# brocksam/pycollo

Measured on AMD Instinct MI355X. Metric: NLP-callback evals/sec (g + jac_g + hess), higher is better.
Workload: dtype f64; 1 GPU; hypersensitive, 1 phase, 2000 mesh sections x 6 Lobatto nodes = 10001 collocation nodes; num_x=20003, num_c=10001, nnz_jac=140003, nnz_hess=20002, tiles=167, threads_per_block=64, waves_per_tile=4, launches_per_eval=1, lds_bytes_per_workgroup=24144, launch_thread_cpu=245, pin_survived_hip_init=True

## Files before the change

pycollo_amd/codegen.py:

```python
from __future__ import annotations

import hashlib
import os
import shutil
import subprocess

import sympy as sym
from sympy.printing.c import C99CodePrinter

from .model import Model, PhaseModel, PointModel

CSRC = os.path.join(os.path.dirname(os.path.abspath(__file__)), "csrc")
CACHE = os.path.join(os.path.dirname(os.path.abspath(__file__)), "_cache")
ARCH = "gfx950"


class _Printer(C99CodePrinter):

    def _print_Pow(self, expr):
        base, exp = expr.base, expr.exp
        b = self.parenthesize(base, 200)
        if exp.is_Integer:
            n = int(exp)
            if n == 0:
# ... 468 lines not shown
        return 2 + len(_static_w_list(model.phases[0], single_phase=True))
    return 3 + len(sorted(set.intersection(*[set(_static_w_list(pm)) for pm in model.phases])))


def part_paths(code_object: str) -> list[str]:
    out, k = [code_object], 1
    while os.path.exists(f"{code_object[:-6]}.p{k}.hsaco"):
        out.append(f"{code_object[:-6]}.p{k}.hsaco")
        k += 1
    return out


def _waves_per_eu() -> int:
    try:
        return int(os.environ.get("PYCOLLO_AMD_WAVES_PER_EU", "0"))
    except ValueError:
        return 0


def _extra_defines() -> list[str]:
    return [d for d in os.environ.get("PYCOLLO_AMD_DEFINES", "").split() if d]


HEAVY_SCRATCH_LIMIT = int(os.environ.get("PYCOLLO_AMD_HEAVY_SCRATCH_LIMIT", "384"))


def _heavy_cap_enabled() -> bool:
    return os.environ.get("PYCOLLO_AMD_HEAVY_CAP", "1") != "0" and _waves_per_eu() == 0


def _heavy_attr(heavy: bool, cap: bool) -> str:
    return "__attribute__((amdgpu_waves_per_eu(2))) " if (heavy and cap) else ""


def _occupancy_attr() -> str:
    w = _waves_per_eu()
    return f"__attribute__((amdgpu_waves_per_eu({w},{w}))) " if w > 0 else ""


def _fp_contract() -> str:
    v = os.environ.get("PYCOLLO_AMD_FP_CONTRACT", "off").strip().lower()
    return v if v in ("off", "fast", "on") else "off"


def _preload_count() -> int:
    try:
        return max(0, int(os.environ.get("PYCOLLO_AMD_PRELOAD", "10")))
    except ValueError:
        return 10


def _kernels_stamp() -> str:
    h = hashlib.sha256()
    for fn in ("pc_kernels.hpp", "pc_solution.hpp", "pc_args.h"):
        with open(os.path.join(CSRC, fn), "rb") as f:
            h.update(f.read())
    with open(os.path.abspath(__file__), "rb") as f:
        h.update(f.read())
    h.update(b"flags:-O3 -ffp-contract=off")
    return h.hexdigest()[:12]


def hipcc_path() -> str | None:
    for cand in (shutil.which("hipcc"), "/opt/rocm/bin/hipcc"):
        if cand and os.path.exists(cand):
            return cand
    return None


def _orders_tag(model: Model, orders, mixed=None) -> str:
    orders = tuple(int(o) for o in orders) if orders is not None else tuple(0 for _ in model.phases)
    if len(orders) != len(model.phases):
        raise ValueError("one section order (or 0) per phase is required")
    tag = "n" + "_".join(str(o) for o in orders)
    mixed = _norm_mixed(model, orders, mixed)
    if any(mixed):
        tag += "-m" + "_".join(".".join(str(n) for n in m) if m else "x" for m in mixed)
    return tag


def code_object_path(model: Model, orders=None, mixed=None) -> str:
    occ = f"_w{_waves_per_eu()}" if _waves_per_eu() > 0 else ""
    if _fp_contract() != "off":
        occ += "_fc" + _fp_contract()
    if _preload_count() != 10:
        occ += f"_pl{_preload_count()}"
    if not _heavy_cap_enabled() and _waves_per_eu() == 0:
        occ += "_nocap"
    if not _heavy_w4_enabled():
        occ += "_nohw4"
    if HEAVY_SCRATCH_LIMIT != 384:
        occ += f"_sl{HEAVY_SCRATCH_LIMIT}"
    if _extra_defines():
        occ += "_d" + hashlib.sha256(" ".join(_extra_defines()).encode()).hexdigest()[:8]
    return os.path.join(CACHE, f"model_{model.digest}_{_kernels_stamp()}_{_orders_tag(model, orders, mixed)}{occ}.hsaco")


def build_code_object(model: Model, orders=None, force: bool = False, verbose: bool = False, mixed=None) -> str:
    os.makedirs(CACHE, exist_ok=True)
    out = code_object_path(model, orders, mixed)
    if os.path.exists(out) and not force:
        return out
    hipcc = hipcc_path()
    if hipcc is None:
        raise RuntimeError(f"code object {out} is not built and hipcc is not available to build it")
    preload = os.environ.get("LD_PRELOAD", "")
    if "rocprof" in preload or any(k.startswith(("ROCPROF", "ROCPROFILER")) for k in os.environ):
# ... 100 lines not shown
```

pycollo_amd/csrc/pc_kernels.hpp:

```cpp
#pragma once

#include <hip/hip_runtime.h>
#include <tuple>
#include <type_traits>
#include <utility>

#include "pc_args.h"

namespace pc {

template <int I>
using ic = std::integral_constant<int, I>;

template <int B, int E, class F>
__device__ __forceinline__ void static_for(F&& f) {
  if constexpr (B < E) {
    f(ic<B>{});
    static_for<B + 1, E>(f);
  }
}

#ifndef PC_SPLIT_MIN
#define PC_SPLIT_MIN 90
#endif

template <class M>
struct S {
  static constexpr int NY = M::NY, NU = M::NU, NZ = M::NY + M::NU, NQ = M::NQ, NP = M::NP, NS = M::NS;
  static constexpr int NT = (M::T0_FREE ? 1 : 0) + (M::TF_FREE ? 1 : 0);
  static constexpr int NFN = NY + NP + NQ, NV = NZ + NS, NJ = M::NJ, NH = M::NH;

  static constexpr int jidx(int r, int c) {
    for (int e = 0; e < NJ; ++e)
      if (M::jr(e) == r && M::jc(e) == c) return e;
    return -1;
  }
  static constexpr bool dep(int r, int c) { return jidx(r, c) >= 0; }
  static constexpr int D(int a) {
    int n = 0;
    for (int b = 0; b < NZ; ++b) n += dep(a, b) ? 1 : 0;
    return n;
  }
  static constexpr int ndep_before(int a, int b) {
    int n = 0;
    for (int bb = 0; bb < b; ++bb) n += dep(a, bb) ? 1 : 0;
    return n;
  }
  static constexpr bool own_sparse(int a) { return !dep(a, a); }
  static constexpr bool is_t(int l) { return M::wk(l) == 2; }
  static constexpr bool is_q(int l) { return M::wk(l) == 1; }
  static constexpr int NWT = [] {
    int n = 0;
    for (int l = 0; l < NS; ++l) n += is_t(l) ? 1 : 0;
    return n;
  }();
  static constexpr int tpar(int jt) {
    for (int l = 0; l < NS; ++l)
      if (is_t(l) && M::wi(l) == jt) return l;
    return -1;
  }
  static constexpr int qpar(int m) {
    for (int l = 0; l < NS; ++l)
      if (is_q(l) && M::wi(l) == m) return l;
    return -1;
  }
  static constexpr int nsdep(int r) {
    int n = 0;
    for (int l = 0; l < NS; ++l) n += dep(r, NZ + l) ? 1 : 0;
    return n;
  }
  static constexpr int srank(int r, int l) {
    int n = 0;
    for (int ll = 0; ll < l; ++ll) n += dep(r, NZ + ll) ? 1 : 0;
    return n;
  }
  static constexpr int nqdep(int r) {
// ... 57 lines not shown
      if (!(r >= NY && r < NY + NP) && dep(r, c)) return true;
    return false;
  }
  static constexpr int hidx(int r, int c) {
    for (int e = 0; e < NH; ++e)
      if (M::hr(e) == r && M::hc(e) == c) return e;
    return -1;
  }
  static constexpr bool tzx(int c) {
    if (tz(c)) return true;
    for (int l = 0; l < NS; ++l)
      if (is_t(l) && hidx(NZ + l, c) >= 0) return true;
    return false;
  }
  static constexpr int erank(int i) {
    int n = 0;
    for (int k = 0; k < i; ++k) n += M::efl(k) ? 1 : 0;
    return n;
  }
  static constexpr int R_Q = 0;
  static constexpr bool has_rts(int l) { return NT > 0 && tz(NZ + l); }
  static constexpr int rqs(int m, int l) {
    int n = NQ;
    for (int mm = 0; mm < NQ; ++mm)
      for (int ll = 0; ll < NS; ++ll) {
        if (mm == m && ll == l) return n;
        n += dep(NY + NP + mm, NZ + ll) ? 1 : 0;
      }
    return n;
  }
  static constexpr int rts(int l) {
    int n = rqs(NQ, 0);
    for (int ll = 0; ll < l; ++ll) n += has_rts(ll) ? 1 : 0;
    return n;
  }
  static constexpr int rss(int l, int l2) {
    int n = rts(NS);
    for (int e = 0; e < NH; ++e)
      if (M::hc(e) >= NZ) {
        if (M::hr(e) == NZ + l && M::hc(e) == NZ + l2) return n;
        ++n;
      }
    return n;
  }
  static constexpr int NRED = rss(NS, NS);
  static constexpr int O_VZ = 0, O_RZ = NZ, O_VQ = 2 * NZ, O_RQ = 2 * NZ + NQ, O_VT = 2 * NZ + 2 * NQ,
                       O_RT = O_VT + 2, O_VS = O_RT + 2, O_RS = O_VS + NS, O_WD = O_RS + NS, O_WP = O_WD + NY,
                       O_WI = O_WP + NP, NSCAL = O_WI + NQ;
  static constexpr int GO_D = 0, GO_P = NY, GO_Q = NY + NP;
  static constexpr int HO_Z = 0, HO_T = NZ, HO_S = 3 * NZ;

  static constexpr int IT_D = 0, IT_P = NY, IT_Q = NY + NP, IT_HB = NY + NP + NQ, IT_HS = IT_HB + NZ,
                       IT_HT = IT_HS + NZ, IT_HSUM = IT_HT + NZ, NITEMS = IT_HSUM + 1;
  struct Deal {
    int own[NITEMS];
    unsigned hmask;
  };
  template <int W, int NN>
  static constexpr Deal deal() {
    Deal d{};
    int wt[NITEMS] = {};
    bool done[NITEMS] = {};
    for (int a = 0; a < NY; ++a) wt[IT_D + a] = D(a) * NN + C(a) + 1;
    for (int m = 0; m < NP; ++m) wt[IT_P + m] = nzdep(NY + m) + nsdep(NY + m) + 1;
    for (int m = 0; m < NQ; ++m) wt[IT_Q + m] = nzdep(NY + NP + m) + 1;
    for (int b = 0; b < NZ; ++b) {
      wt[IT_HB + b] = hrow_count(b) > 0 ? hrow_count(b) + 1 : 0;
      int ns = 0;
      for (int e = 0; e < NH; ++e) ns += (M::hr(e) >= NZ && !is_t(M::hr(e) - NZ) && M::hc(e) == b) ? 1 : 0;
      wt[IT_HS + b] = ns;
      wt[IT_HT + b] = tzx(b) ? NT : 0;
    }
    wt[IT_HSUM] = NS > 0 ? NS + NS * (NS + 1) / 2 : 0;
    int load[W] = {};
    d.hmask = 0;
    for (int it = 0; it < NITEMS; ++it) {
      int best = -1;
      for (int i = 0; i < NITEMS; ++i)
        if (!done[i] && (best < 0 || wt[i] > wt[best])) best = i;
      done[best] = true;
      const bool hess = best >= IT_HB;
      int bin = hess ? W - 1 : 0;
      for (int k = 0; k < W; ++k) {
        const int b = hess ? W - 1 - k : k;
        if (load[b] < load[bin]) bin = b;
      }
      d.own[best] = wt[best] > 0 ? bin : 0;
      load[bin] += wt[best];
      if (hess && wt[best] > 0) d.hmask |= 1u << bin;
    }
    return d;
  }
  static constexpr int red_item(int r) {
    if (r < NQ) return IT_Q + r;
    for (int m = 0; m < NQ; ++m)
      for (int l = 0; l < NS; ++l)
        if (dep(NY + NP + m, NZ + l) && rqs(m, l) == r) return IT_Q + m;
    return IT_HSUM;
  }
};


template <int CTRL>
__device__ __forceinline__ double dpp_mov(double v) {
  const long long b = __builtin_bit_cast(long long, v);
  const int lo = __builtin_amdgcn_update_dpp(0, (int)(b & 0xffffffffll), CTRL, 0xf, 0xf, true);
  const int hi = __builtin_amdgcn_update_dpp(0, (int)(b >> 32), CTRL, 0xf, 0xf, true);
  return __builtin_bit_cast(double, ((long long)(unsigned)hi << 32) | (long long)(unsigned)lo);
}
__device__ __forceinline__ double wave_sum(double v) {
  v += dpp_mov<0x111>(v);
  v += dpp_mov<0x112>(v);
  v += dpp_mov<0x114>(v);
  v += dpp_mov<0x118>(v);
  const long long b = __builtin_bit_cast(long long, v);
  double tot = 0.0;
#pragma unroll
  for (int r = 0; r < 4; ++r) {
    const int lo = __builtin_amdgcn_readlane((int)(b & 0xffffffffll), 16 * r + 15);
    const int hi = __builtin_amdgcn_readlane((int)(b >> 32), 16 * r + 15);
    tot += __builtin_bit_cast(double, ((long long)(unsigned)hi << 32) | (long long)(unsigned)lo);
  }
  return tot;
}

__device__ __forceinline__ void lds_barrier() {
  asm volatile("s_waitcnt lgkmcnt(0)\n\ts_barrier" ::: "memory");
}

typedef double pc_d2_a8 __attribute__((ext_vector_type(2), aligned(8)));
#ifndef PC_FLUSH_DEPTH
#define PC_FLUSH_DEPTH 4
#endif
typedef int pc_i4 __attribute__((ext_vector_type(4)));
__device__ __forceinline__ void flush_run(double* __restrict__ dst, const double* __restrict__ src, int len, int tid,
                                          int TB) {
  len = __builtin_amdgcn_readfirstlane(len);
  if (len <= 0) return;
  const unsigned long long d64 = (unsigned long long)dst;
  double* base = (double*)(((unsigned long long)(unsigned)__builtin_amdgcn_readfirstlane((int)(d64 >> 32)) << 32) |
                           (unsigned long long)(unsigned)__builtin_amdgcn_readfirstlane((int)d64));
  __amdgpu_buffer_rsrc_t rs = __builtin_amdgcn_make_buffer_rsrc(base, 0, len * 8, 0x00020000);
  const int pairs = (len + 1) >> 1;
  const pc_d2_a8* sp = reinterpret_cast<const pc_d2_a8*>(src) + tid;
// ... 9 lines not shown
  }
  if (b0 < pairs) {
    pc_d2_a8 a[PC_FLUSH_DEPTH];
#pragma unroll
    for (int q = 0; q < PC_FLUSH_DEPTH; ++q) a[q] = sp[b0 + q * TB];
#pragma unroll
    for (int q = 0; q < PC_FLUSH_DEPTH; ++q)
      if (b0 + q * TB < pairs)
        __builtin_amdgcn_raw_buffer_store_b128(__builtin_bit_cast(pc_i4, a[q]), rs, voff + q * TB * 16, 0, 0);
  }
}

template <int L, int GS>
__device__ __forceinline__ void flush_chunks(double* __restrict__ dst, const double* __restrict__ src, int nq, int t, int TN) {
  nq = __builtin_amdgcn_readfirstlane(nq);
  if (nq <= 0) return;
  if (TN == 64) {
    constexpr int NR = (L + 127) / 128;
    const unsigned long long d64 = (unsigned long long)dst;
    double* base = (double*)(((unsigned long long)(unsigned)__builtin_amdgcn_readfirstlane((int)(d64 >> 32)) << 32) |
                             (unsigned long long)(unsigned)__builtin_amdgcn_readfirstlane((int)d64));
    const double* sp = src + 2 * t;
    const int voff = 16 * t;
    pc_d2_a8 a[NR], nx[NR];
    auto fetch = [&](pc_d2_a8* r, const double* p) {
#pragma unroll
      for (int i = 0; i < NR; ++i) r[i] = *reinterpret_cast<const pc_d2_a8*>(p + 128 * i);
    };
    auto store = [&](const pc_d2_a8* r, double* b) {
      __amdgpu_buffer_rsrc_t rs = __builtin_amdgcn_make_buffer_rsrc(b, 0, L * 8, 0x00020000);
#pragma unroll
      for (int i = 0; i < NR; ++i) __builtin_amdgcn_raw_buffer_store_b128(__builtin_bit_cast(pc_i4, r[i]), rs, voff + 1024 * i, 0, 0);
    };
    fetch(a, sp);
    int q = 0;
    for (; q + 2 <= nq; q += 2) {
      fetch(nx, sp + L);
      store(a, base);
      if (q + 2 < nq) fetch(a, sp + 2 * L);
      store(nx, base + GS);
      sp += 2 * L;
      base += 2 * GS;
    }
    if (q < nq) store(a, base);
    return;
  }
  for (int q = 0; q < nq; ++q) {
    const double* sp = src + (long long)q * L;
    double* dp = dst + (long long)q * GS;
    for (int o = 2 * t; o < L; o += 2 * TN) {
      if (o + 1 < L) *reinterpret_cast<pc_d2_a8*>(dp + o) = *reinterpret_cast<const pc_d2_a8*>(sp + o);
      else dp[o] = sp[o];
    }
  }
}

template <class St>
struct BulkIn {
  const double* x; const double* lam; double* c; double* G; double* H;
  const double* xz; const double* lamd;
  const int32_t* tile_k0; const int32_t* tile_n0; const int32_t* sec_s; const double* sec_h; const int64_t* sec_E;
  const double* qa; const double* qw; const int64_t* hslot0; const int64_t* hslotN; double* partials;
  unsigned long long* gran; unsigned long long* erec; const double* tab;
  int64_t x_off, s_off, c_off, c_path_off, c_int_off;
  double t_fixed[2];
  int32_t N, K, flags, qa_total, qw_total, tile_begin, uni_n, spt, lds_out, wpt, n_blocks, block_threads, qa0, qw0, qwabs;
  uint32_t epoch;
  int32_t erec0;
  double scal[St::NSCAL > 0 ? St::NSCAL : 1];
  int64_t goff[St::NFN > 0 ? St::NFN : 1];
  int64_t hoff[3 * St::NZ + St::NS * St::NZ > 0 ? 3 * St::NZ + St::NS * St::NZ : 1];
};

#ifndef PC_PIN_BUDGET
#define PC_PIN_BUDGET 40
#endif
template <class T>
__device__ __forceinline__ uintptr_t pin_word(T* v) { return reinterpret_cast<uintptr_t>(v); }
__device__ __forceinline__ unsigned long long pin_word(double v) { return __builtin_bit_cast(unsigned long long, v); }
__device__ __forceinline__ long long pin_word(long long v) { return v; }
__device__ __forceinline__ long pin_word(long v) { return v; }
__device__ __forceinline__ int pin_word(int v) { return v; }
template <class... T>
__device__ __forceinline__ auto pin_vals(const T&... v) { return std::make_tuple(pin_word(v)...); }
template <bool C, class... T>
__device__ __forceinline__ auto pin_if(const T&... v) {
  if constexpr (C) return pin_vals(v...);
  else return std::tuple<>{};
}
template <class Pred, class T, int N, int... I>
__device__ __forceinline__ auto pin_array_impl(const T (&a)[N], std::integer_sequence<int, I...>) {
  return std::tuple_cat(pin_if<Pred::test(I)>(a[I])...);
}
struct PinEvery { static constexpr bool test(int) { return true; } };
template <int CNT, class Pred, class T, int N>
__device__ __forceinline__ auto pin_array_where(const T (&a)[N]) {
  return pin_array_impl<Pred>(a, std::make_integer_sequence<int, CNT>{});
}
template <int CNT, class T, int N>
__device__ __forceinline__ auto pin_array(const T (&a)[N]) { return pin_array_where<CNT, PinEvery>(a); }
#define PC_PIN_OP(i) "s"(std::get<i>(g))
#define PC_PIN_OPS_1 PC_PIN_OP(0)
#define PC_PIN_OPS_2 PC_PIN_OPS_1, PC_PIN_OP(1)
#define PC_PIN_OPS_3 PC_PIN_OPS_2, PC_PIN_OP(2)
#define PC_PIN_OPS_4 PC_PIN_OPS_3, PC_PIN_OP(3)
#define PC_PIN_OPS_5 PC_PIN_OPS_4, PC_PIN_OP(4)
// ... 261 lines not shown
      if (odd_prev) r_cp = tid < r_nprev - 1 ? A.qa[r_qaprev + tid * r_nprev + r_nprev - 1] : 0.0;
    }
  };
  const bool early_aux = LD != nullptr && UN > 0 && !MIX;
  if (early_aux) aux_loads();
  const auto first_group = std::tuple_cat(
      pin_vals(A.x, A.lam, A.sec_h, A.qa, A.qw, A.x_off, A.c_off, A.N, A.K, A.flags, A.qa_total, A.qw_total, A.tile_begin,
               A.uni_n, A.spt, A.lds_out, A.wpt, A.n_blocks, A.block_threads),
      pin_if<(UN > 0)>(A.qa0, A.qwabs), pin_if<(NP > 0)>(A.c_path_off), pin_if<(NQ > 0)>(A.c_int_off), pin_if<(NS > 0)>(A.s_off),
      pin_if<UN == 0>(A.tile_k0, A.tile_n0, A.sec_s, A.sec_E));
  if (early_aux) pin_group<true>(first_group);
  else pin_group(first_group);
  constexpr int NHO = 3 * NZ + NS * NZ;
  constexpr bool PINNED = 2 * (St::NSCAL + NFN + NHO) <= PC_PIN_BUDGET;
  struct ScalUsed {
    static constexpr bool test(int i) {
      return (i < St::O_VQ) || (i >= St::O_VT && i < St::O_VT + St::NT) || (i >= St::O_RT && i < St::O_RT + St::NT) || (i >= St::O_VS);
    }
  };
  struct HoffUsed {
    static constexpr bool test(int i) { return i < St::NZ || (St::NT > 0 && i < 3 * St::NZ) || i >= 3 * St::NZ; }
  };
  auto pin_second_group = [&]() {
    auto outs = std::tuple_cat(pin_vals(A.c, A.G, A.H), pin_if<(NRED > 0 && RES)>(A.gran), pin_if<(NRED > 0 && !RES)>(A.partials),
                               pin_if<!M::T0_FREE>(A.t_fixed[0]), pin_if<!M::TF_FREE>(A.t_fixed[1]));
    if constexpr (PINNED) {
      pin_group(std::tuple_cat(outs, pin_array_where<St::NSCAL, ScalUsed>(A.scal), pin_array<NFN>(A.goff),
                               pin_array_where<NHO, HoffUsed>(A.hoff)));
    } else {
      pin_group(std::tuple_cat(outs, pin_vals(A.tab)));
    }
  };

  extern __shared__ double smem[];
  const int TN = W > 1 ? 64 : TB;
  const int w = WN > 0 ? WIDX : (W > 1 ? __builtin_amdgcn_readfirstlane(tid >> 6) : 0);
  const LdsPlan lp = lds_plan(TN, A.qa_total, A.qw_total, NY, NFS, NRED, A.lds_out * W, St::NSCAL + NFN + 3 * NZ + NS * NZ, UN == 0, MIX);
  double* s_cp = smem + lp.cp;
  double* s_qa = smem + lp.qa;
  double* s_qw = smem + lp.qw;
  int* s_off = reinterpret_cast<int*>(smem + lp.off);
  auto QAO = [&](int n) -> int { return UN > 0 ? 0 : s_off[n]; };
  auto QWO = [&](int n) -> int { return UN > 0 ? 0 : s_off[PC_MAX_ORDER + 1 + n]; };
  double* s_h = smem + lp.h;
  long long* s_E = reinterpret_cast<long long*>(smem + lp.E);
  int* s_s = reinterpret_cast<int*>(smem + lp.s);
  int* s_kr = reinterpret_cast<int*>(smem + lp.kr);
  double* s_f = smem + lp.f;
  double* s_yu = smem + lp.yu;
  double* s_fs = smem + lp.fs;
  double* s_lam = smem + lp.lam;
  double* s_red = smem + lp.red;
  double* s_out = smem + lp.out + w * A.lds_out;
  constexpr auto DEAL2 = St::template deal<2, (UN > 0 ? UN : 4)>();
  constexpr auto DEAL4 = St::template deal<4, (UN > 0 ? UN : 4)>();
  auto mine = [&](auto item_) -> bool {
    constexpr int item = decltype(item_)::value;
    return W == 1 || (W == 2 ? DEAL2.own[item] : DEAL4.own[item]) == w;
  };
  const bool hess_replica = W == 1 || (((W == 2 ? DEAL2.hmask : DEAL4.hmask) >> w) & 1u);
#define PC_ITEM(i) std::integral_constant<int, (i)>{}
#ifndef PC_WAVE_FENCE
#define PC_WAVE_FENCE() asm volatile("" ::: "memory")
#endif
  const bool one_wave = (TB == 64);
  const bool wave_private = one_wave || W > 1;
  auto stage_sync = [&]() {
    if (wave_private) PC_WAVE_FENCE();
    else lds_barrier();
  };
  auto block_sync = [&]() {
    if (one_wave) PC_WAVE_FENCE();
    else lds_barrier();
  };
  auto node_sync = [&]() {
    if (wave_private) PC_WAVE_FENCE();
    else lds_barrier();
  };

  const bool wantC = A.flags & PC_FLAG_C, wantG = A.flags & PC_FLAG_G;

  const bool last_tile = (k1 == A.K);

  double* s_tab = smem + lp.tab;
  const double* sc;
  const int64_t* goff;
  const int64_t* hoff;
  if constexpr (PINNED) {
    sc = A.scal;
    goff = A.goff;
    hoff = A.hoff;
  } else {
    sc = s_tab;
    goff = reinterpret_cast<const int64_t*>(s_tab + St::NSCAL);
    hoff = goff + NFN;
  }
  const bool owns = active && (t < T || last_tile);
  double F[NFN > 0 ? NFN : 1], Jv[NJ > 0 ? NJ : 1], Hv[NH > 0 ? NH : 1], mu[NFN > 0 ? NFN : 1];
  double red[NRED > 0 ? NRED : 1];
  static_for<0, NRED>([&](auto r_) { red[decltype(r_)::value] = 0.0; });
  if (active) {
    static_for<0, NS>([&](auto l_) {
      constexpr int l = decltype(l_)::value;
      constexpr int kind = M::wk(l), idx = M::wi(l);
      v[NZ + l] = A.x[kind == 0 ? A.s_off + idx : A.x_off + (int64_t)NZ * N + (kind == 1 ? idx : NQ + idx)];
    });
  }
  double lam_p[NP > 0 ? NP : 1], lam_q[NQ > 0 ? NQ : 1];
  if (owns && wantH && hess_replica) {
    static_for<0, NP>([&](auto m_) { lam_p[decltype(m_)::value] = A.lam[A.c_path_off + (int64_t) decltype(m_)::value * N + node]; });
    static_for<0, NQ>([&](auto m_) { lam_q[decltype(m_)::value] = A.lam[A.c_int_off + decltype(m_)::value]; });
// ... 71 lines not shown

  double t0 = A.t_fixed[0], tF = A.t_fixed[1];
  double dst[2] = {0.0, 0.0};
  {
    const int64_t t_off = A.x_off + (int64_t)NZ * N + NQ;
    int j = 0;
    if constexpr (M::T0_FREE) {
      t0 = sc[St::O_VT + j] * A.x[t_off + j] + sc[St::O_RT + j];
      dst[j] = -0.5 * sc[St::O_VT + j];
      ++j;
    }
    if constexpr (M::TF_FREE) {
      tF = sc[St::O_VT + j] * A.x[t_off + j] + sc[St::O_RT + j];
      dst[j] = 0.5 * sc[St::O_VT + j];
    }
  }
  const double stretch = 0.5 * (tF - t0);

  int ls_r = -1, pos_r = 0, n_r = UN > 0 ? UN : 2, ls_s = 0, n_s = UN > 0 ? UN : 2;
  bool has_start = false;
  double w_node = 0.0;
  const bool prev_lane = odd_prev && t == 0;
  if (active) {
    static_for<0, NZ>([&](auto b_) {
      constexpr int b = decltype(b_)::value;
      v[b] = sc[St::O_VZ + b] * v[b] + sc[St::O_RZ + b];
    });
    static_for<0, NS>([&](auto l_) {
      constexpr int l = decltype(l_)::value;
      v[NZ + l] = sc[St::O_VS + l] * v[NZ + l] + sc[St::O_RS + l];
    });
    PC_STAMP(1);
    if constexpr (PURE) {
      ls_r = t == 0 ? lsA - 1 : lsA + (t - 1) / (UN - 1);
    } else if (uni) {
      const int g = node - kp * (un - 1);
      ls_r = (node == 0) ? -1 : (g - 1) / (un - 1);
    } else {
      ls_r = s_kr[t];
    }
    ls_s = ls_r + 1;
    has_start = (node < N - 1) && (ls_s < nsec) && (S_s(ls_s) == node);
    if (ls_r >= 0) {
      n_r = S_n(ls_r);
      pos_r = node - S_s(ls_r);
      w_node = prev_lane ? S_h(ls_r) * r_wprev : S_h(ls_r) * s_qw[QWO(n_r) + (prev_lane ? 0 : pos_r)];
    }
    if (has_start) {
      n_s = S_n(ls_s);
      w_node += S_h(ls_s) * s_qw[QWO(n_s)];
    }
  }

#ifndef PC_HOIST_MAX
#define PC_HOIST_MAX 8
#endif
  constexpr bool HOIST = (UN > 0 && UN <= PC_HOIST_MAX);
  constexpr int NC = HOIST ? UN - 1 : 1;
  double cr[NC], cs[NC];
  if constexpr (HOIST) {
#pragma unroll
    for (int j = 0; j < NC; ++j) cr[j] = cs[j] = 0.0;
    if (active) {
      const double* At = s_qa + QAO(UN);
      if (ls_r >= 0 && !prev_lane) {
        const double h = S_h(ls_r);
#pragma unroll
        for (int j = 1; j < UN; ++j) cr[j - 1] = h * At[(j - 1) * UN + pos_r];
      }
      if (has_start) {
        const double h = S_h(ls_s);
#pragma unroll
        for (int j = 1; j < UN; ++j) cs[j - 1] = h * At[(j - 1) * UN];
      }
    }
  }

  static_for<0, NFN>([&](auto r_) { mu[decltype(r_)::value] = 0.0; });
  if (owns && wantH && hess_replica) {
    static_for<0, NY>([&](auto a_) {
      constexpr int a = decltype(a_)::value;
      const double* la = s_lam + a * (TN + PC_MAX_ORDER);
      double acc = 0.0;
      if constexpr (PURE) {
        if (prev_lane) {
          double a2 = 0.0;
          for (int j = 0; j < r_nprev - 1; ++j) a2 += la[j] * s_cp[j];
          acc += S_h(0) * a2;
        }
      }
      if constexpr (HOIST) {
        if (ls_r >= 0 && !prev_lane) {
          const int base = S_s(ls_r) - lam0;
#pragma unroll
          for (int j = 1; j < UN; ++j) acc += la[base + j - 1] * cr[j - 1];
        }
        if (has_start) {
          const int base = S_s(ls_s) - lam0;
          double a2 = 0.0;
#pragma unroll
          for (int j = 1; j < UN; ++j) a2 += la[base + j - 1] * cs[j - 1];
          acc += a2;
        }
      } else {
        if (ls_r >= 0 && !prev_lane) {
          const double* At = s_qa + QAO(n_r);
          const int base = S_s(ls_r) - lam0;
          double a2 = 0.0;
#pragma unroll
// ... 159 lines not shown
  if constexpr (RED_EARLY) deposit_partials();
  PC_STAMP(2);
  node_sync();

  double accf[NY > 0 ? NY : 1];
  const bool rowthr = active && t >= 1;
#ifdef PC_MFMA_DEFECT
  constexpr bool MFMA_DEF = UN > 0 && NY > 0 && NY <= 16;
  double accm[NY > 0 ? NY : 1];
  bool mfma_done = false;
  if constexpr (MFMA_DEF) {
    if (TN == 64 && (wantC || wantG)) {
      typedef double pc_d4 __attribute__((ext_vector_type(4)));
      constexpr int n = UN > 0 ? UN : 2;
      constexpr int KS = (16 + 2 * (n - 1) + 1 + 3) / 4;
      const int lane = t & 63, q = lane & 15, hq = lane >> 4;
      const double* Atab = s_qa + QAO(n);
      static_for<0, NY>([&](auto a_) { accm[decltype(a_)::value] = 0.0; });
#pragma unroll
      for (int g = 0; g < 4; ++g) {
        if (16 * g >= T) break;
        const int rr = 16 * g + q;
        const int sec = rr / (n - 1), jm1 = rr - sec * (n - 1), sk = sec * (n - 1);
        const int kb = ((16 * g) / (n - 1)) * (n - 1);
        pc_d4 acc4 = {0.0, 0.0, 0.0, 0.0};
#pragma unroll
        for (int s4 = 0; s4 < KS; ++s4) {
          const int kk = kb + 4 * s4 + hq;
          const int i = kk - sk;
          const bool in = rr < T && i >= 0 && i < n;
          const double coef = Atab[in ? jm1 * n + i : 0];
          const double fval = s_f[min(q, NY - 1) * TN + min(kk, T)];
          acc4 = __builtin_amdgcn_mfma_f64_16x16x4f64(q < NY ? fval : 0.0, in ? coef : 0.0, acc4, 0, 0, 0);
        }
        const int mine_q = (t - 1) & 15;
        const bool here = rowthr && ((t - 1) >> 4) == g;
        static_for<0, NY>([&](auto a_) {
          constexpr int a = decltype(a_)::value;
          const double got = __shfl(acc4[a >> 2], 16 * (a & 3) + mine_q, 64);
          if (here) accm[a] = got;
        });
      }
      mfma_done = true;
    }
  }
#endif
  if (rowthr && (wantC || wantG)) {
    const int n = UN > 0 ? UN : n_r, j = pos_r, sk = S_s(ls_r) - n0;
    const double h = S_h(ls_r);
    const double* Arow = s_qa + QAO(n) + (j - 1) * n;
    static_for<0, NY>([&](auto a_) {
      constexpr int a = decltype(a_)::value;
      accf[a] = 0.0;
      if (!mine(PC_ITEM(St::IT_D + a))) return;
      double acc = 0.0;
#ifdef PC_MFMA_DEFECT
      if (mfma_done) {
        acc = accm[a];
      } else
#endif
      {
#pragma unroll
        for (int i = 0; i < n; ++i) acc += Arow[i] * s_f[a * TN + sk + i];
      }
      accf[a] = h * acc;
      if (wantC)
        A.c[A.c_off + (int64_t)a * (N - 1) + node - 1] = sc[St::O_WD + a] * ((s_yu[a * TN + sk] - v[a]) + stretch * accf[a]);
    });
  }
  PC_STAMP(3);
  block_sync();

  static_for<0, NP>([&](auto m_) {
    constexpr int m = decltype(m_)::value;
    constexpr int r = NY + m;
    constexpr int R = PC_CE(St::nzdep(r)) + PC_CE(St::nsdep(r));
    const double Wp = sc[St::O_WP + m];
    if (owns && wantC && mine(PC_ITEM(St::IT_P + m))) A.c[A.c_path_off + (int64_t)m * N + node] = Wp * F[r];
    if (wantG && R > 0 && mine(PC_ITEM(St::IT_P + m))) {
      if (owns) {
        static_for<0, NZ>([&](auto b_) {
          constexpr int b = decltype(b_)::value;
          if constexpr (PC_CE(St::dep(r, b))) s_out[t * R + PC_CE(St::zrank(r, b))] = Wp * sc[St::O_VZ + b] * Jv[PC_CE(St::jidx(r, b))];
        });
        static_for<0, NS>([&](auto l_) {
          constexpr int l = decltype(l_)::value;
          if constexpr (PC_CE(St::dep(r, NZ + l)))
            s_out[t * R + PC_CE(St::nzdep(r)) + PC_CE(St::srank(r, l))] = Wp * sc[St::O_VS + l] * Jv[PC_CE(St::jidx(r, NZ + l))];
        });
      }
      stage_sync();
      flush_run(A.G + goff[St::GO_P + m] + (int64_t)n0 * R, s_out, n_own * R, t, TN);
      stage_sync();
    }
  });

  if (owns) {
    static_for<0, NQ>([&](auto m_) {
      constexpr int m = decltype(m_)::value;
      constexpr int r = NY + NP + m;
      if (wantG && mine(PC_ITEM(St::IT_Q + m))) {
        const double k = -sc[St::O_WI + m] * stretch * w_node;
        static_for<0, NZ>([&](auto b_) {
          constexpr int b = decltype(b_)::value;
          if constexpr (PC_CE(St::dep(r, b)))
            A.G[goff[St::GO_Q + m] + (int64_t)PC_CE(St::zrank(r, b)) * N + node] = k * sc[St::O_VZ + b] * Jv[PC_CE(St::jidx(r, b))];
        });
      }
    });
  }

  auto hess_tstrips = [&]() {
    if (owns) {
      if constexpr (NT > 0) {
        static_for<0, NV>([&](auto c_) {
          constexpr int cvar = decltype(c_)::value;
          if constexpr (cvar < NZ ? PC_CE(St::tzx(cvar)) : PC_CE(St::tz(cvar))) {
            double acc = 0.0;
            static_for<0, NFN>([&](auto r_) {
              constexpr int r = decltype(r_)::value;
              if constexpr (!(r >= NY && r < NY + NP) && PC_CE(St::dep(r, cvar))) acc += mu[r] * Jv[PC_CE(St::jidx(r, cvar))];
            });
            if constexpr (cvar < NZ) {
              if (mine(PC_ITEM(St::IT_HT + cvar))) static_for<0, NT>([&](auto j_) {
                constexpr int j = decltype(j_)::value;
                double* dstp = A.H + hoff[St::HO_T + j * NZ + cvar] + node;
                double val = dst[j] * sc[St::O_VZ + cvar] * acc;
                constexpr int lt = PC_CE(St::tpar(j));
                if constexpr (lt >= 0) {
                  constexpr int eh = PC_CE(St::hidx(NZ + (lt >= 0 ? lt : 0), cvar));
                  if constexpr (eh >= 0) val += sc[St::O_VS + lt] * sc[St::O_VZ + cvar] * Hv[eh];
                }
                if (edge0 || edgeN) edge_store(ic<St::NHZZ + j * NZ + cvar>{}, dstp, val); else *dstp = val;
              });
            } else {
              red[PC_CE(St::rts(cvar - NZ))] = acc;
            }
          }
        });
      }
    }
  };
  if (wantH && hess_replica) {
    if constexpr (!SPLIT) hess_second();
    hess_tstrips();
  }

  if constexpr (!SPLIT && !RED_EARLY) deposit_partials();
  PC_STAMP(4);
  if (wantG) {
    auto uniform64 = [](long long v) -> long long {
      const unsigned lo = __builtin_amdgcn_readfirstlane((unsigned)(unsigned long long)v);
      const unsigned hi = __builtin_amdgcn_readfirstlane((unsigned)((unsigned long long)v >> 32));
      return (long long)(((unsigned long long)hi << 32) | lo);
    };
    const long long E0 = uni ? S_E(lsA) : uniform64(S_E(lsA)), E1 = uni ? S_E(nsec) : uniform64(S_E(nsec));
    constexpr int RSTRIDE_MAX = [] {
      int m = 0;
      for (int a = 0; a < NY; ++a) m = St::D(a) * (UN > 0 ? UN : 0) + St::C(a) > m ? St::D(a) * (UN > 0 ? UN : 0) + St::C(a) : m;
      return m;
    }();
    constexpr int NPASS = (UN > 0 && WN != 4) ? pc_row_passes(UN, RSTRIDE_MAX) : 1;
    constexpr int RG = UN > 0 ? (UN - 1 + NPASS - 1) / NPASS : 0;
    auto defect_jacobian_of_state = [&](auto a_) {
      constexpr int a = decltype(a_)::value;
      if (!mine(PC_ITEM(St::IT_D + a))) return;
      constexpr int Da = St::D(a), Ca = St::C(a);
      const double Wd = sc[St::O_WD + a];
      auto row_off = [&](int ls, int j, int n) -> int {
        const int eloc = uni ? (ls - lsA) * (n - 1) * n : (int)(S_E(ls) - E0);
        return Da * eloc + Ca * (S_s(ls) - n0) + (j - 1) * (Da * n + Ca);
      };
      double js[Da > 0 ? Da : 1];
      const double WS = Wd * stretch, WV = Wd * sc[St::O_VZ + a];
      if (active) {
        static_for<0, NZ>([&](auto b_) {
          constexpr int b = decltype(b_)::value;
          if constexpr (PC_CE(St::dep(a, b))) js[PC_CE(St::ndep_before(a, b))] = WS * (Jv[PC_CE(St::jidx(a, b))] * sc[St::O_VZ + b]);
        });
      }
      auto param_cols = [&](int rs) {
        if constexpr (NT + PC_CE(St::nxdep(a)) > 0) {
          const int n = UN > 0 ? UN : n_r, jr = pos_r, sk = S_s(ls_r) - n0;
          auto dfdw = [&](auto l_) -> double {
            constexpr int l = decltype(l_)::value;
            const double* Arow = s_qa + QAO(n) + (jr - 1) * n;
            double as = 0.0;
#pragma unroll
            for (int i = 0; i < n; ++i) as += Arow[i] * s_fs[PC_CE(St::fs_slot(a, l)) * TN + sk + i];
            return Wd * stretch * sc[St::O_VS + l] * (S_h(ls_r) * as);
          };
          static_for<0, NT>([&](auto jt_) {
            constexpr int jt = decltype(jt_)::value;
            double val = Wd * dst[jt] * accf[a];
            constexpr int lt = PC_CE(St::tpar(jt));
            if constexpr (lt >= 0) {
              if constexpr (PC_CE(St::dep(a, NZ + (lt >= 0 ? lt : 0)))) val += dfdw(ic<(lt >= 0 ? lt : 0)>{});
            }
            s_out[rs + PC_CE(St::nqdep(a)) + jt] = val;
          });
          static_for<0, NS>([&](auto l_) {
            constexpr int l = decltype(l_)::value;
            if constexpr (!St::is_t(l) && PC_CE(St::dep(a, NZ + l))) s_out[rs + PC_CE(St::xpos(a, l))] = dfdw(l_);
          });
        }
      };
      const int64_t g0 = goff[St::GO_D + a] + (int64_t)Da * E0 + (int64_t)Ca * n0;
      if constexpr (NPASS > 1) {
        constexpr int RS = Da * UN + Ca;
        static_for<0, NPASS>([&](auto g_) {
          constexpr int g = decltype(g_)::value;
          constexpr int JLO = 1 + g * RG, JHI = (JLO + RG < UN) ? JLO + RG : UN, RGG = JHI - JLO;
          if constexpr (RGG > 0) {
            if (active) {
              auto write_cols = [&](int ls, int pos, const double* cc) {
                const double h = HOIST ? 0.0 : S_h(ls);
                const double* At = s_qa;
                const int rs0 = (ls - lsA) * (RGG * RS);
                static_for<JLO, JHI>([&](auto j_) {
                  constexpr int jj = decltype(j_)::value;
                  const double coef = HOIST ? cc[jj - 1] : h * At[(jj - 1) * UN + pos];
                  static_for<0, NZ>([&](auto b_) {
                    constexpr int b = decltype(b_)::value;
                    if constexpr (PC_CE(St::dep(a, b))) {
                      constexpr int before = PC_CE(St::ndep_before(a, b));
                      constexpr int extra = (PC_CE(St::own_sparse(a)) && a < b) ? 2 : 0;
                      double val = coef * js[before];
                      if constexpr (a == b) val += WV * ((pos == 0 ? 1.0 : 0.0) - (pos == jj ? 1.0 : 0.0));
                      s_out[rs0 + (jj - JLO) * RS + before * UN + extra + pos] = val;
                    }
                  });
                });
              };
              if (ls_r >= lsA) write_cols(ls_r, pos_r, cr);
              if (has_start) write_cols(ls_s, 0, cs);
              if (t >= 1 && pos_r >= JLO && pos_r < JHI) {
                const int rs = (ls_r - lsA) * (RGG * RS) + (pos_r - JLO) * RS;
                if constexpr (PC_CE(St::own_sparse(a))) {
                  s_out[rs + PC_CE(St::ndep_before(a, a)) * UN] = WV;
                  s_out[rs + PC_CE(St::ndep_before(a, a)) * UN + 1] = -WV;
                }
                param_cols(rs + Da * UN + (PC_CE(St::own_sparse(a)) ? 2 : 0));
              }
            }
            stage_sync();
            flush_chunks<RGG * RS, (UN - 1) * RS>(A.G + g0 + (JLO - 1) * RS, s_out, k1 - k0, t, TN);
            stage_sync();
          }
        });
        if constexpr (a < 7) PC_STAMP(11 + 2 * a);
        return;
      }
      if (active) {
        auto write_cols = [&](int ls, int pos, int n_in, const double* cc) {
          const int n = UN > 0 ? UN : n_in;
          const double h = HOIST ? 0.0 : S_h(ls);
          const double* At = s_qa + (HOIST ? 0 : QAO(n));
          const int rs1 = row_off(ls, 1, n), rstride = Da * n + Ca;
#pragma unroll
          for (int j = 1; j < n; ++j) {
            const double coef = HOIST ? cc[j - 1] : h * At[(j - 1) * n + pos];
            const int rs = rs1 + (j - 1) * rstride;
            static_for<0, NZ>([&](auto b_) {
              constexpr int b = decltype(b_)::value;
              if constexpr (PC_CE(St::dep(a, b))) {
                constexpr int before = PC_CE(St::ndep_before(a, b));
                constexpr int extra = (PC_CE(St::own_sparse(a)) && a < b) ? 2 : 0;
                double val = coef * js[before];
                if constexpr (a == b) val += WV * ((pos == 0 ? 1.0 : 0.0) - (pos == j ? 1.0 : 0.0));
                s_out[rs + before * n + extra + pos] = val;
              }
            });
          }
        };
        if (ls_r >= lsA) write_cols(ls_r, pos_r, n_r, cr);
        if (has_start) write_cols(ls_s, 0, n_s, cs);
        if constexpr (PC_CE(St::own_sparse(a))) {
          if (t >= 1) {
            const int n = UN > 0 ? UN : n_r;
            const int o = row_off(ls_r, pos_r, n) + PC_CE(St::ndep_before(a, a)) * n;
            s_out[o] = WV;
            s_out[o + 1] = -WV;
          }
        }
        if (rowthr) {
          const int n = UN > 0 ? UN : n_r;
          param_cols(row_off(ls_r, pos_r, n) + Da * n + (PC_CE(St::own_sparse(a)) ? 2 : 0));
        }
      }
      stage_sync();
      if constexpr (a < 7) PC_STAMP(10 + 2 * a);
      const int len = (int)((long long)Da * (E1 - E0)) + Ca * T;
      flush_run(A.G + g0, s_out, len, t, TN);
      stage_sync();
      if constexpr (a < 7) PC_STAMP(11 + 2 * a);
    };
    static_for<0, NY>(defect_jacobian_of_state);
  }

  PC_STAMP(5);
  if constexpr (SPLIT) {
    second_pass();
    if constexpr (!RED_EARLY) deposit_partials();
  }
// ... 429 lines not shown
```

Measured before the change: 244,500 evals/s.

## Split heavy defect-Jacobian rows across wave replicas and add packed buffer-store flush

Moves the compile-time work-dealing logic into a new header and extends it so that a dominant state's defect-Jacobian item can be cut into up to two row groups, each owned by a different wave replica. This targets load imbalance when one state's Jacobian block dominates the per-tile work. Split groups are flushed through a new packed 128-bit buffer-store routine that spreads short chunks evenly across lanes. The cost is extra LDS syncs per group and duplicated defect accumulation on every wave that owns a group.

```diff
diff --git a/pycollo_amd/codegen.py b/pycollo_amd/codegen.py
--- a/pycollo_amd/codegen.py
+++ b/pycollo_amd/codegen.py
@@ -544,7 +544,7 @@
 
 def _kernels_stamp() -> str:
     h = hashlib.sha256()
-    for fn in ("pc_kernels.hpp", "pc_solution.hpp", "pc_args.h"):
+    for fn in ("pc_kernels.hpp", "pc_deal.hpp", "pc_solution.hpp", "pc_args.h"):
         with open(os.path.join(CSRC, fn), "rb") as f:
             h.update(f.read())
     with open(os.path.abspath(__file__), "rb") as f:
diff --git a/pycollo_amd/csrc/pc_deal.hpp b/pycollo_amd/csrc/pc_deal.hpp
--- /dev/null
+++ b/pycollo_amd/csrc/pc_deal.hpp
@@ -0,0 +1,79 @@
+#pragma once
+
+namespace pcd {
+
+constexpr int MAX_W = 4;
+
+#ifndef PC_DEAL_GROUPS_MAX
+#define PC_DEAL_GROUPS_MAX 2
+#endif
+
+template <int NITEMS, int NY>
+struct Deal {
+  static constexpr int NYA = NY > 0 ? NY : 1;
+  int own[NITEMS];
+  unsigned hmask;
+  int ng[NYA];
+  int lo[NYA][MAX_W];
+  int hi[NYA][MAX_W];
+  int gown[NYA][MAX_W];
+  int gwt[NYA][MAX_W];
+  int load[MAX_W];
+};
+
+template <int W, int NITEMS, int NY>
+constexpr Deal<NITEMS, NY> deal(const int (&wt)[NITEMS], int first_hess, int rows) {
+  static_assert(W >= 1 && W <= MAX_W, "replicas per tile");
+  Deal<NITEMS, NY> d{};
+  int total = 0;
+  for (int i = 0; i < NITEMS; ++i) total += wt[i];
+  constexpr int NE = NITEMS + Deal<NITEMS, NY>::NYA * (MAX_W - 1);
+  int ew[NE] = {}, eitem[NE] = {}, egrp[NE] = {};
+  bool done[NE] = {};
+  int ne = 0;
+  for (int it = 0; it < NITEMS; ++it) {
+    if (it >= NY) {
+      ew[ne] = wt[it], eitem[ne] = it, egrp[ne] = 0, ++ne;
+      continue;
+    }
+    int G = 1;
+    if (rows >= 2 && total > 0 && wt[it] * W >= 2 * total) {
+      G = wt[it] * W / total;
+      if (G > rows) G = rows;
+      if (G > W) G = W;
+      if (G > PC_DEAL_GROUPS_MAX) G = PC_DEAL_GROUPS_MAX;
+      if (G < 1) G = 1;
+    }
+    d.ng[it] = G;
+    int j = 1;
+    for (int g = 0; g < G; ++g) {
+      const int r = G == 1 ? rows : rows / G + (g < rows % G ? 1 : 0);
+      d.lo[it][g] = j;
+      d.hi[it][g] = j + r;
+      j += r;
+      d.gwt[it][g] = G == 1 ? wt[it] : ((wt[it] - 1) * r + rows - 1) / rows + (g == 0 ? 1 : 0);
+      ew[ne] = d.gwt[it][g], eitem[ne] = it, egrp[ne] = g, ++ne;
+    }
+  }
+  d.hmask = 0;
+  for (int n = 0; n < ne; ++n) {
+    int best = -1;
+    for (int i = 0; i < ne; ++i)
+      if (!done[i] && (best < 0 || ew[i] > ew[best])) best = i;
+    done[best] = true;
+    const bool hess = eitem[best] >= first_hess;
+    int bin = hess ? W - 1 : 0;
+    for (int k = 0; k < W; ++k) {
+      const int b = hess ? W - 1 - k : k;
+      if (d.load[b] < d.load[bin]) bin = b;
+    }
+    const int owner = ew[best] > 0 ? bin : 0;
+    if (egrp[best] == 0) d.own[eitem[best]] = owner;
+    if (eitem[best] < NY) d.gown[eitem[best]][egrp[best]] = owner;
+    d.load[bin] += ew[best];
+    if (hess && ew[best] > 0) d.hmask |= 1u << bin;
+  }
+  return d;
+}
+
+}
diff --git a/pycollo_amd/csrc/pc_kernels.hpp b/pycollo_amd/csrc/pc_kernels.hpp
--- a/pycollo_amd/csrc/pc_kernels.hpp
+++ b/pycollo_amd/csrc/pc_kernels.hpp
@@ -6,6 +6,7 @@
 #include <utility>
 
 #include "pc_args.h"
+#include "pc_deal.hpp"
 
 namespace pc {
 
@@ -22,6 +23,9 @@
 
 #ifndef PC_SPLIT_MIN
 #define PC_SPLIT_MIN 90
+#endif
+#ifndef PC_HOIST_MAX
+#define PC_HOIST_MAX 8
 #endif
 
 template <class M>
@@ -185,15 +189,10 @@
 
   static constexpr int IT_D = 0, IT_P = NY, IT_Q = NY + NP, IT_HB = NY + NP + NQ, IT_HS = IT_HB + NZ,
                        IT_HT = IT_HS + NZ, IT_HSUM = IT_HT + NZ, NITEMS = IT_HSUM + 1;
-  struct Deal {
-    int own[NITEMS];
-    unsigned hmask;
-  };
-  template <int W, int NN>
+  using Deal = pcd::Deal<NITEMS, NY>;
+  template <int W, int NN, bool CUT = false>
   static constexpr Deal deal() {
-    Deal d{};
     int wt[NITEMS] = {};
-    bool done[NITEMS] = {};
     for (int a = 0; a < NY; ++a) wt[IT_D + a] = D(a) * NN + C(a) + 1;
     for (int m = 0; m < NP; ++m) wt[IT_P + m] = nzdep(NY + m) + nsdep(NY + m) + 1;
     for (int m = 0; m < NQ; ++m) wt[IT_Q + m] = nzdep(NY + NP + m) + 1;
@@ -205,24 +204,7 @@
       wt[IT_HT + b] = tzx(b) ? NT : 0;
     }
     wt[IT_HSUM] = NS > 0 ? NS + NS * (NS + 1) / 2 : 0;
-    int load[W] = {};
-    d.hmask = 0;
-    for (int it = 0; it < NITEMS; ++it) {
-      int best = -1;
-      for (int i = 0; i < NITEMS; ++i)
-        if (!done[i] && (best < 0 || wt[i] > wt[best])) best = i;
-      done[best] = true;
-      const bool hess = best >= IT_HB;
-      int bin = hess ? W - 1 : 0;
-      for (int k = 0; k < W; ++k) {
-        const int b = hess ? W - 1 - k : k;
-        if (load[b] < load[bin]) bin = b;
-      }
-      d.own[best] = wt[best] > 0 ? bin : 0;
-      load[bin] += wt[best];
-      if (hess && wt[best] > 0) d.hmask |= 1u << bin;
-    }
-    return d;
+    return pcd::deal<W, NITEMS, NY>(wt, IT_HB, CUT ? NN - 1 : 0);
   }
   static constexpr int red_item(int r) {
     if (r < NQ) return IT_Q + r;
@@ -338,6 +320,31 @@
       if (o + 1 < L) *reinterpret_cast<pc_d2_a8*>(dp + o) = *reinterpret_cast<const pc_d2_a8*>(sp + o);
       else dp[o] = sp[o];
     }
+  }
+}
+
+template <int L, int GS>
+__device__ __forceinline__ void flush_chunks_packed(double* __restrict__ dst, const double* __restrict__ src, int nq, int t) {
+  static_assert(L % 2 == 0 && L < 128 && GS >= L, "short even chunks only");
+  nq = __builtin_amdgcn_readfirstlane(nq);
+  if (nq <= 0) return;
+  constexpr int PL = L / 2;
+  const unsigned long long d64 = (unsigned long long)dst;
+  double* base = (double*)(((unsigned long long)(unsigned)__builtin_amdgcn_readfirstlane((int)(d64 >> 32)) << 32) |
+                           (unsigned long long)(unsigned)__builtin_amdgcn_readfirstlane((int)d64));
+  __amdgpu_buffer_rsrc_t rs = __builtin_amdgcn_make_buffer_rsrc(base, 0, ((nq - 1) * GS + L) * 8, 0x00020000);
+  const int pairs = nq * PL;
+  const pc_d2_a8* sp = reinterpret_cast<const pc_d2_a8*>(src) + t;
+  for (int b0 = 0; b0 < pairs; b0 += PC_FLUSH_DEPTH * 64) {
+    pc_d2_a8 a[PC_FLUSH_DEPTH];
+#pragma unroll
+    for (int q = 0; q < PC_FLUSH_DEPTH; ++q) a[q] = sp[b0 + q * 64];
+#pragma unroll
+    for (int q = 0; q < PC_FLUSH_DEPTH; ++q)
+      if (b0 + q * 64 < pairs) {
+        const int p = b0 + q * 64 + t, ch = p / PL;
+        __builtin_amdgcn_raw_buffer_store_b128(__builtin_bit_cast(pc_i4, a[q]), rs, (ch * GS + 2 * (p - ch * PL)) * 8, 0, 0);
+      }
   }
 }
 
@@ -705,11 +712,33 @@
   double* s_lam = smem + lp.lam;
   double* s_red = smem + lp.red;
   double* s_out = smem + lp.out + w * A.lds_out;
-  constexpr auto DEAL2 = St::template deal<2, (UN > 0 ? UN : 4)>();
-  constexpr auto DEAL4 = St::template deal<4, (UN > 0 ? UN : 4)>();
-  auto mine = [&](auto item_) -> bool {
+  constexpr int RSTRIDE_MAX = [] {
+    int m = 0;
+    for (int a = 0; a < NY; ++a) m = St::D(a) * (UN > 0 ? UN : 0) + St::C(a) > m ? St::D(a) * (UN > 0 ? UN : 0) + St::C(a) : m;
+    return m;
+  }();
+  constexpr int NPASS = (UN > 0 && WN != 4) ? pc_row_passes(UN, RSTRIDE_MAX) : 1;
+  constexpr int RG = UN > 0 ? (UN - 1 + NPASS - 1) / NPASS : 0;
+  constexpr bool CUT = UN > 0 && UN <= PC_HOIST_MAX && NPASS == 1;
+  constexpr auto DEAL2 = St::template deal<2, (UN > 0 ? UN : 4), CUT>();
+  constexpr auto DEAL4 = St::template deal<4, (UN > 0 ? UN : 4), CUT>();
+  auto mine = [&](auto item_, auto... g_) -> bool {
     constexpr int item = decltype(item_)::value;
-    return W == 1 || (W == 2 ? DEAL2.own[item] : DEAL4.own[item]) == w;
+    if constexpr (sizeof...(g_) > 0) {
+      constexpr int g = (0 + ... + decltype(g_)::value);
+      return W == 1 || (W == 2 ? DEAL2.gown[item][g] : DEAL4.gown[item][g]) == w;
+    } else {
+      return W == 1 || (W == 2 ? DEAL2.own[item] : DEAL4.own[item]) == w;
+    }
+  };
+  auto mine_any = [&](auto a_) -> bool {
+    constexpr int a = decltype(a_)::value;
+    bool any = mine(ic<St::IT_D + a>{});
+    static_for<1, pcd::MAX_W>([&](auto g_) {
+      constexpr int g = decltype(g_)::value;
+      if ((W == 2 && g < DEAL2.ng[a]) || (W == 4 && g < DEAL4.ng[a])) any = any || mine(ic<St::IT_D + a>{}, g_);
+    });
+    return any;
   };
   const bool hess_replica = W == 1 || (((W == 2 ? DEAL2.hmask : DEAL4.hmask) >> w) & 1u);
 #define PC_ITEM(i) std::integral_constant<int, (i)>{}
@@ -887,9 +916,6 @@
     }
   }
 
-#ifndef PC_HOIST_MAX
-#define PC_HOIST_MAX 8
-#endif
   constexpr bool HOIST = (UN > 0 && UN <= PC_HOIST_MAX);
   constexpr int NC = HOIST ? UN - 1 : 1;
   double cr[NC], cs[NC];
@@ -1155,7 +1181,7 @@
     static_for<0, NY>([&](auto a_) {
       constexpr int a = decltype(a_)::value;
       accf[a] = 0.0;
-      if (!mine(PC_ITEM(St::IT_D + a))) return;
+      if (!mine_any(a_)) return;
       double acc = 0.0;
 #ifdef PC_MFMA_DEFECT
       if (mfma_done) {
@@ -1167,7 +1193,7 @@
         for (int i = 0; i < n; ++i) acc += Arow[i] * s_f[a * TN + sk + i];
       }
       accf[a] = h * acc;
-      if (wantC)
+      if (wantC && mine(PC_ITEM(St::IT_D + a)))
         A.c[A.c_off + (int64_t)a * (N - 1) + node - 1] = sc[St::O_WD + a] * ((s_yu[a * TN + sk] - v[a]) + stretch * accf[a]);
     });
   }
@@ -1258,16 +1284,9 @@
       return (long long)(((unsigned long long)hi << 32) | lo);
     };
     const long long E0 = uni ? S_E(lsA) : uniform64(S_E(lsA)), E1 = uni ? S_E(nsec) : uniform64(S_E(nsec));
-    constexpr int RSTRIDE_MAX = [] {
-      int m = 0;
-      for (int a = 0; a < NY; ++a) m = St::D(a) * (UN > 0 ? UN : 0) + St::C(a) > m ? St::D(a) * (UN > 0 ? UN : 0) + St::C(a) : m;
-      return m;
-    }();
-    constexpr int NPASS = (UN > 0 && WN != 4) ? pc_row_passes(UN, RSTRIDE_MAX) : 1;
-    constexpr int RG = UN > 0 ? (UN - 1 + NPASS - 1) / NPASS : 0;
     auto defect_jacobian_of_state = [&](auto a_) {
       constexpr int a = decltype(a_)::value;
-      if (!mine(PC_ITEM(St::IT_D + a))) return;
+      if (!mine_any(a_)) return;
       constexpr int Da = St::D(a), Ca = St::C(a);
       const double Wd = sc[St::O_WD + a];
       auto row_off = [&](int ls, int j, int n) -> int {
@@ -1309,50 +1328,76 @@
         }
       };
       const int64_t g0 = goff[St::GO_D + a] + (int64_t)Da * E0 + (int64_t)Ca * n0;
+      auto row_group = [&](auto jlo_, auto jhi_, auto dealt_) {
+        constexpr int RS = Da * UN + Ca;
+        constexpr int JLO = decltype(jlo_)::value, JHI = decltype(jhi_)::value, RGG = JHI - JLO;
+        constexpr bool DEALT = decltype(dealt_)::value;
+        if constexpr (RGG > 0) {
+          if (active) {
+            auto write_cols = [&](int ls, int pos, const double* cc) {
+              const double h = HOIST ? 0.0 : S_h(ls);
+              const double* At = s_qa;
+              const int rs0 = (ls - lsA) * (RGG * RS);
+              static_for<JLO, JHI>([&](auto j_) {
+                constexpr int jj = decltype(j_)::value;
+                const double coef = HOIST ? cc[jj - 1] : h * At[(jj - 1) * UN + pos];
+                static_for<0, NZ>([&](auto b_) {
+                  constexpr int b = decltype(b_)::value;
+                  if constexpr (PC_CE(St::dep(a, b))) {
+                    constexpr int before = PC_CE(St::ndep_before(a, b));
+                    constexpr int extra = (PC_CE(St::own_sparse(a)) && a < b) ? 2 : 0;
+                    double val = coef * js[before];
+                    if constexpr (a == b) val += WV * ((pos == 0 ? 1.0 : 0.0) - (pos == jj ? 1.0 : 0.0));
+                    s_out[rs0 + (jj - JLO) * RS + before * UN + extra + pos] = val;
+                  }
+                });
+              });
+            };
+            if (ls_r >= lsA) write_cols(ls_r, pos_r, cr);
+            if (has_start) write_cols(ls_s, 0, cs);
+            if (t >= 1 && pos_r >= JLO && pos_r < JHI) {
+              const int rs = (ls_r - lsA) * (RGG * RS) + (pos_r - JLO) * RS;
+              if constexpr (PC_CE(St::own_sparse(a))) {
+                s_out[rs + PC_CE(St::ndep_before(a, a)) * UN] = WV;
+                s_out[rs + PC_CE(St::ndep_before(a, a)) * UN + 1] = -WV;
+              }
+              param_cols(rs + Da * UN + (PC_CE(St::own_sparse(a)) ? 2 : 0));
+            }
+          }
+          stage_sync();
+          if constexpr (DEALT && a < 7) PC_STAMP(10 + 2 * a);
+          constexpr int L = RGG * RS, GS = (UN - 1) * RS;
+          if constexpr (DEALT && L % 2 == 0 && L < 128) flush_chunks_packed<L, GS>(A.G + g0 + (JLO - 1) * RS, s_out, k1 - k0, t);
+          else flush_chunks<L, GS>(A.G + g0 + (JLO - 1) * RS, s_out, k1 - k0, t, TN);
+          stage_sync();
+        }
+      };
       if constexpr (NPASS > 1) {
-        constexpr int RS = Da * UN + Ca;
         static_for<0, NPASS>([&](auto g_) {
           constexpr int g = decltype(g_)::value;
-          constexpr int JLO = 1 + g * RG, JHI = (JLO + RG < UN) ? JLO + RG : UN, RGG = JHI - JLO;
-          if constexpr (RGG > 0) {
-            if (active) {
-              auto write_cols = [&](int ls, int pos, const double* cc) {
-                const double h = HOIST ? 0.0 : S_h(ls);
-                const double* At = s_qa;
-                const int rs0 = (ls - lsA) * (RGG * RS);
-                static_for<JLO, JHI>([&](auto j_) {
-                  constexpr int jj = decltype(j_)::value;
-                  const double coef = HOIST ? cc[jj - 1] : h * At[(jj - 1) * UN + pos];
-                  static_for<0, NZ>([&](auto b_) {
-                    constexpr int b = decltype(b_)::value;
-                    if constexpr (PC_CE(St::dep(a, b))) {
-                      constexpr int before = PC_CE(St::ndep_before(a, b));
-                      constexpr int extra = (PC_CE(St::own_sparse(a)) && a < b) ? 2 : 0;
-                      double val = coef * js[before];
-                      if constexpr (a == b) val += WV * ((pos == 0 ? 1.0 : 0.0) - (pos == jj ? 1.0 : 0.0));
-                      s_out[rs0 + (jj - JLO) * RS + before * UN + extra + pos] = val;
-                    }
-                  });
-                });
-              };
-              if (ls_r >= lsA) write_cols(ls_r, pos_r, cr);
-              if (has_start) write_cols(ls_s, 0, cs);
-              if (t >= 1 && pos_r >= JLO && pos_r < JHI) {
-                const int rs = (ls_r - lsA) * (RGG * RS) + (pos_r - JLO) * RS;
-                if constexpr (PC_CE(St::own_sparse(a))) {
-                  s_out[rs + PC_CE(St::ndep_before(a, a)) * UN] = WV;
-                  s_out[rs + PC_CE(St::ndep_before(a, a)) * UN + 1] = -WV;
-                }
-                param_cols(rs + Da * UN + (PC_CE(St::own_sparse(a)) ? 2 : 0));
-              }
-            }
-            stage_sync();
-            flush_chunks<RGG * RS, (UN - 1) * RS>(A.G + g0 + (JLO - 1) * RS, s_out, k1 - k0, t, TN);
-            stage_sync();
-          }
+          constexpr int JLO = 1 + g * RG, JHI = (JLO + RG < UN) ? JLO + RG : UN;
+          row_group(ic<JLO>{}, ic<JHI>{}, std::false_type{});
         });
         if constexpr (a < 7) PC_STAMP(11 + 2 * a);
         return;
+      }
+      if constexpr (CUT) {
+        constexpr int G2 = DEAL2.ng[a], G4 = DEAL4.ng[a];
+        if constexpr (G2 > 1 || G4 > 1) {
+          if (W == 4 ? G4 > 1 : (W == 2 && G2 > 1)) {
+            static_for<0, pcd::MAX_W>([&](auto g_) {
+              constexpr int g = decltype(g_)::value;
+              if constexpr (g < G4) {
+                if (W == 4 && mine(PC_ITEM(St::IT_D + a), g_)) row_group(ic<DEAL4.lo[a][g]>{}, ic<DEAL4.hi[a][g]>{}, std::true_type{});
+              }
+              if constexpr (g < G2) {
+                if (W == 2 && mine(PC_ITEM(St::IT_D + a), g_)) row_group(ic<DEAL2.lo[a][g]>{}, ic<DEAL2.hi[a][g]>{}, std::true_type{});
+              }
+            });
+            if constexpr (a < 7) PC_STAMP(11 + 2 * a);
+            return;
+          }
+        }
       }
       if (active) {
         auto write_cols = [&](int ls, int pos, int n_in, const double* cc) {
```

After: 237,800 evals/s. -2.7%, worse.
